# 1314wu/kvazaar

Hardware: AMD Instinct MI355X
Metric: Mblocks/s (SAD8/SATD8/DCT32) per GPU (higher is better)
Workload: dtype u8

## Files before the change

kvazaar_amd/csrc/api.hip:

```cpp
#include "kvz_hip_internal.h"

#include <atomic>
#include <cstdio>
#include <cstdlib>
#include <cstring>
#include <string>
#include <mutex>

namespace kvzhip {

constexpr int KVZ_MAX_DEVICES = 64;
struct dev_ctx {
  std::atomic<bool> ready{false};
  int num_cus = 256;
  hipStream_t stream = nullptr;
  char name[256] = "";
};
static std::mutex g_mu;
static dev_ctx g_ctx[KVZ_MAX_DEVICES];
static std::atomic<int> g_default_dev{-1};
static thread_local int t_dev = -1;
static thread_local char g_err[512] = "";

struct tune_entry { const char *key; std::atomic<int> value; };
static tune_entry g_tune[] = { { "sad_wgs_per_cu", {-1} }, { "satd8_wgs_per_cu", {-1} }, { "dct32_wgs_per_cu", {-1} },
                               { "idct32_wgs_per_cu", {-1} }, { "dct_wgs_per_cu", {-1} }, { "qr32_wgs_per_cu", {-1} },
                               { "qr_wgs_per_cu", {-1} }, { "dct16_wgs_per_cu", {-1} }, { "idct16_wgs_per_cu", {-1} },
                               { "qr16_wgs_per_cu", {-1} }, { "qr4_lane_kernel", {-1} },
                               { "sao_edge_fast", {-1} }, 
                               { "intra_rough_waves", {-1} }, { "pair_wave_kernel", {-1} }, { "qr4_wgs_per_cu", {-1} }, { "quant_wgs_per_cu", {-1} },
                               { "qr8_reg_kernel", {-1} }, { "qr8_wgs_per_cu", {-1} }, { "qr_tile_kernel", {-1} }, { "dct4_tile", {-1} }, { "dct4_wgs_per_cu", {-1} }, { "idct4_wgs_per_cu", {-1} },
                               { "wg_chunk_min_wgs", {-1} }, { "pair_satd_threads", {-1} }, { "qr8_tile_kernel", {-1} }, { "qr_tile_pipe", {-1} }, { "pipe", {-1} }, { "dct_pipe", {-1} }, { "sample8_wave", {-1} }, { "full_qsad", {-1} }, { "service_streams", {-1} }, { "service_inflight", {-1} }, { "service_workers", {-1} }, { "service_linger_us", {-1} }, { "service_life_ms", {-1} }, { "service_spin_us", {-1} }, { "service_ticket_base_k", {-1} }, { "service_push", {-1} }, { "service_nap_us", {-1} }, { "service_spin_crowded_us", {-1} } };
int tuning(const char *key, int dflt)
{
  for (auto &e : g_tune) if (!std::strcmp(e.key, key)) { const int v = e.value.load(std::memory_order_relaxed); return v >= 0 ? v : dflt; }
  return dflt;
}

int ctx_device() { return t_dev >= 0 ? t_dev : g_default_dev.load(std::memory_order_acquire); }
bool ctx_ready()
{
  const int d = ctx_device();
  return d >= 0 && g_ctx[d].ready.load(std::memory_order_acquire);
}

bool ctx_enter()
{
  const int d = ctx_device();
  if (d < 0 || !g_ctx[d].ready.load(std::memory_order_acquire)) return false;
  int cur = -1;
  if (hipGetDevice(&cur) != hipSuccess || cur != d) {
    if (hipSetDevice(d) != hipSuccess) return false;
  }
  return true;
}
// ... 390 lines not shown
```

kvazaar_amd/csrc/frac_core.h:

```cpp
#pragma once
#include "kvz_hip_internal.h"
#include "satd_regs.h"

namespace kvzhip {

static __constant__ __attribute__((aligned(8))) signed char c_luma_filter[4][8] = {
  { 0, 0, 0, 64, 0, 0, 0, 0 }, { -1, 4, -10, 58, 17, -5, 1, 0 }, { -1, 4, -11, 40, 40, -11, 4, -1 }, { 0, 1, -5, 17, 58, -10, 4, -1 } };

struct refplane_t { const u8 *p; u32 stride; int w, h; };

__device__ __forceinline__ u8 ref_px(const refplane_t &r, int x, int y)
{
  return r.p[(size_t)clampi(y, 0, r.h - 1) * r.stride + clampi(x, 0, r.w - 1)];
}

__device__ __forceinline__ u8 round_clip16(i16 sample) { return fast_clip16((i16)(((int)sample + 32) >> 6)); }

#define FR_HS 65

static __constant__ signed char c_sq_x[9] = { 0, -1, 1, 0, 0, -1, 1, -1, 1 };
static __constant__ signed char c_sq_y[9] = { 0, 0, 0, -1, 1, -1, -1, 1, 1 };

template <int MAXW>
struct frac_geom {
// ... 7 lines not shown
  static constexpr int H_OFF = (P_BYTES + CUR_BYTES + 15) & ~15;
  static constexpr int TOTAL = H_OFF + 4 * H_ELEMS * 2 + 32;
};

struct frac_vcoef { u32 c[4][2][2][5]; };
__host__ __device__ constexpr u32 frac_pack16(int lo, int hi) { return ((u32)lo & 0xffffu) | ((u32)hi << 16); }
__host__ __device__ constexpr frac_vcoef frac_make_vcoef()
{
  constexpr int f[4][8] = { { 0, 0, 0, 256, 0, 0, 0, 0 }, { -4, 16, -40, 232, 68, -20, 4, 0 }, { -4, 16, -44, 160, 160, -44, 16, -4 },
                            { 0, 4, -20, 68, 232, -40, 16, -4 } };
  frac_vcoef t = {};
  for (int fy = 0; fy < 4; ++fy)
    for (int i = 0; i < 5; ++i) {
      const u32 aligned = i < 4 ? frac_pack16(f[fy][2 * i], f[fy][2 * i + 1]) : 0u;
      const u32 shifted = frac_pack16(i > 0 ? f[fy][2 * i - 1] : 0, i < 4 ? f[fy][2 * i] : 0);
      const u32 late = i > 0 ? frac_pack16(f[fy][2 * i - 2], f[fy][2 * i - 1]) : 0u;
      t.c[fy][0][0][i] = aligned; t.c[fy][0][1][i] = shifted;
      t.c[fy][1][0][i] = shifted; t.c[fy][1][1][i] = late;
    }
  return t;
}
static __constant__ const frac_vcoef c_frac_vcoef = frac_make_vcoef();

__device__ __forceinline__ v2s frac_round_clip_pair(int acc_even, int acc_odd)
{
  const v2s sft = as_v2s(__builtin_amdgcn_perm((u32)acc_odd, (u32)acc_even, 0x06050201u));
  const v2s r32 = { 32, 32 }, six = { 6, 6 }, zero = { 0, 0 }, top = { 255, 255 };
  v2s t = __builtin_elementwise_add_sat(sft, r32) >> six;
  t = __builtin_elementwise_max(t, zero);
  return __builtin_elementwise_min(t, top);
}

struct frac_no_cost {
  __device__ __forceinline__ u32 cost(int, int, int, u32 &bits) const { bits = 0; return 0; }
  __device__ __forceinline__ bool within(int, int) const { return true; }
};
struct frac_result { int mvx, mvy; u32 cost, bitcost; u32 cost0; };

template <int MAXW, int T, bool WAVE, class MVC, int FW = 0, int FH = 0>
__device__ __forceinline__ frac_result search_frac_core(int tid, u8 *lds, const u8 *__restrict__ pic, u32 pic_stride, const refplane_t &ref,
                                                        const kvz_hip_block_pair &d, int fme_level, const MVC &mvc,
                                                        u32 *__restrict__ out, i32 *__restrict__ best)
{
  typedef frac_geom<MAXW> G;
  u8 *s_p = lds, *s_cur = s_p + G::P_BYTES;
  u32 *s_h = (u32 *)(lds + G::H_OFF);
  u32 *s_cost = s_h + 4 * (G::H_ELEMS / 2);
  int *s_sel = (int *)(s_cost + 4);
  auto sync = [&]() { if (WAVE) wave_lds_fence(); else __syncthreads(); };

  const int w = FW ? FW : d.width, h = FH ? FH : d.height;
  const int pw = w + 8, ph = h + 8;
  if (d.x2 - 4 >= 0 && d.x2 + w + 4 <= ref.w && d.y2 - 4 >= 0 && d.y2 + h + 4 <= ref.h) {
    const int pw4 = pw >> 2;
    const u8 *src = ref.p + (size_t)(d.y2 - 4) * ref.stride + (d.x2 - 4);
    for (int i = tid; i < pw4 * ph; i += T) {
      const int y = i / pw4, x = (i - y * pw4) * 4;
      u32 v;
      __builtin_memcpy(&v, src + (size_t)y * ref.stride + x, 4);
      *(u32 *)(s_p + y * G::PS + x) = v;
    }
  } else {
    for (int i = tid; i < pw * ph; i += T) {
      const int y = i / pw, x = i - y * pw;
      s_p[y * G::PS + x] = ref_px(ref, d.x2 - 4 + x, d.y2 - 4 + y);
// ... 112 lines not shown
#pragma unroll
      for (int j = 0; j < 8; ++j) {
        const u32 *cj = col + j * (G::HT >> 1);
        a0[j] = 0; a1[j] = 0;
#pragma unroll
        for (int t = 0; t < 5; ++t) {
          const v2s pr = as_v2s(cj[t]);
          a0[j] = __builtin_amdgcn_sdot2(pr, as_v2s(c0[t]), a0[j], false);
          a1[j] = __builtin_amdgcn_sdot2(pr, as_v2s(c1[t]), a1[j], false);
        }
      }
      v2s dd[2][4];
#pragma unroll
      for (int jj = 0; jj < 4; ++jj) {
        const u32 cw0 = cur[jj >> 1], cw1 = cur[2 + (jj >> 1)];
        dd[0][jj] = ((jj & 1) ? unpack_hi(cw0) : unpack_lo(cw0)) - frac_round_clip_pair(a0[2 * jj], a0[2 * jj + 1]);
        dd[1][jj] = ((jj & 1) ? unpack_hi(cw1) : unpack_lo(cw1)) - frac_round_clip_pair(a1[2 * jj], a1[2 * jj + 1]);
      }
      add_cost(k, satd8_quad_part_diff(dd, m1, m2));
    }
    sync();
  };

  auto score_step8 = [&](int pat, int ox, int oy, int scale) {
    const int g = tid & 3, pp = (tid >> 2) & 3, k = tid >> 4;
    const int sx = (int)((0x8858u >> (2 * (pat + k - 1))) & 3u) - 1, sy = (int)((0xa085u >> (2 * (pat + k - 1))) & 3u) - 1;
    const int qx = ox + scale * sx, qy = oy + scale * sy;
    const int fx = qx & 3, fy = qy & 3, cx = qx >> 2, ry = qy >> 2;
    const int slot = fx == 0 ? 0 : fx == 2 ? 1 : (sx > 0 ? 3 : 2);
    const int y0 = 2 * pp, b = y0 + ry + 1, par = b & 1;
    u32 c0[5], c1[5];
#pragma unroll
    for (int t = 0; t < 5; ++t) { c0[t] = c_frac_vcoef.c[fy][par][0][t]; c1[t] = c_frac_vcoef.c[fy][par][1][t]; }
    const u32 *col = s_h + slot * (G::H_ELEMS / 2) + ((2 * g + cx + 1) * G::HT >> 1) + (b >> 1);
    int a0[2], a1[2];
#pragma unroll
    for (int j = 0; j < 2; ++j) {
      const u32 *cj = col + j * (G::HT >> 1);
      a0[j] = 0; a1[j] = 0;
#pragma unroll
      for (int t = 0; t < 5; ++t) {
        const v2s pr = as_v2s(cj[t]);
        a0[j] = __builtin_amdgcn_sdot2(pr, as_v2s(c0[t]), a0[j], false);
        a1[j] = __builtin_amdgcn_sdot2(pr, as_v2s(c1[t]), a1[j], false);
      }
    }
    const u8 *a = s_cur + y0 * G::CS + 2 * g;
    const u32 cw0 = *(const unsigned short *)a, cw1 = *(const unsigned short *)(a + G::CS);
    const v2s r0 = unpack_lo(cw0) - frac_round_clip_pair(a0[0], a0[1]), r1 = unpack_lo(cw1) - frac_round_clip_pair(a1[0], a1[1]);
    const short s4 = (tid & 4) ? (short)-1 : (short)1, s8 = (tid & 8) ? (short)-1 : (short)1;
    const v2s m4 = { s4, s4 }, m8 = { s8, s8 };
    v2s v[2] = { r0 + r1, r0 - r1 };
    u32 acc = 0;
#pragma unroll
    for (int i = 0; i < 2; ++i) {
      v2s t = dpp_v2s<0xB1>(v[i]);
      v2s u = v[i] * m1 + t;
      t = dpp_v2s<0x4E>(u);
      u = u * m2 + t;
      t = dpp_xor4_v2s(u);
      u = u * m4 + t;
      t = dpp_v2s<0x128>(u);
      u = u * m8 + t;
      acc = abs_last_stage(u, acc);
    }
    acc = group_sum<16>(acc);
    if ((tid & 15) == 0) s_cost[k] = (acc + 2) >> 2;
    sync();
  };
  constexpr bool SPLIT8 = WAVE && T == 64 && FW == 8 && FH == 8;
  constexpr bool SPLIT16 = WAVE && T == 64 && FW == 16 && FH == 16;
  auto score_any = [&](int pat, int ox, int oy, int scale) {
    if constexpr (SPLIT8) score_step8(pat, ox, oy, scale); else score_step(pat, ox, oy, scale);
  };

  if constexpr (SPLIT8 || SPLIT16) {
    const int g = tid & 3, pp = (tid >> 2) & 3, sb = SPLIT16 ? tid >> 4 : 0, y0 = (sb >> 1) * 8 + 2 * pp, x0 = (sb & 1) * 8 + 2 * g;
    const u8 *a = s_cur + y0 * G::CS + x0, *bq = s_p + (4 + y0) * G::PS + 4 + x0;
    const u32 cw0 = *(const unsigned short *)a, cw1 = *(const unsigned short *)(a + G::CS);
    const u32 pw0 = *(const unsigned short *)bq, pw1 = *(const unsigned short *)(bq + G::PS);
    const v2s r0 = unpack_lo(cw0) - unpack_lo(pw0), r1 = unpack_lo(cw1) - unpack_lo(pw1);
    const short s4 = (tid & 4) ? (short)-1 : (short)1, s8 = (tid & 8) ? (short)-1 : (short)1;
    const v2s m4 = { s4, s4 }, m8 = { s8, s8 };
    v2s v[2] = { r0 + r1, r0 - r1 };
    u32 acc = 0;
#pragma unroll
    for (int i = 0; i < 2; ++i) {
      v2s t = dpp_v2s<0xB1>(v[i]);
      v2s u = v[i] * m1 + t;
      t = dpp_v2s<0x4E>(u);
      u = u * m2 + t;
      t = dpp_xor4_v2s(u);
      u = u * m4 + t;
      t = dpp_v2s<0x128>(u);
      u = u * m8 + t;
      acc = abs_last_stage(u, acc);
    }
    acc = (group_sum<16>(acc) + 2) >> 2;
    if (SPLIT16) acc = group_sum<64>((tid & 15) == 0 ? acc : 0u);
    if (tid == 0) s_cost[0] = acc;
    sync();
  } else {
    score_integer();
  }
  int mx = d.x2 - d.x1, my = d.y2 - d.y1;
  u32 best_bitcost = 0;
  u32 best_cost = s_cost[0];
  if (out && tid == 0) out[0] = best_cost;
  best_cost += mvc.cost(mx, my, 2, best_bitcost);
  const u32 cost0 = best_cost;
  mx *= 2; my *= 2;

  if (fme_level > 0) hor_planes(0, 0, 2, 1);
  sync();

  int best_index = 0, pat = 1;
  for (int step = 0; step < fme_level; ++step) {
    if (step < 2) {
      score_any(pat, 0, 0, 2);
    } else {
      const int hx = s_sel[0], hy = s_sel[1];
      if (step == 2) {
        hor_planes((2 * hx - 1) & 3, 2, (2 * hx + 1) & 3, 3);
        sync();
      }
      score_any(pat, 2 * hx, 2 * hy, 1);
    }
    const int mv_shift = step < 2 ? 1 : 0;
    const int lj = tid & 3;
    const int lpx = mx + (int)((0x8858u >> (2 * (pat + lj - 1))) & 3u) - 1, lpy = my + (int)((0xa085u >> (2 * (pat + lj - 1))) & 3u) - 1;
    u32 lbits = 0;
    const u32 lraw = s_cost[lj];
    const int lok = mvc.within(lpx * (1 << mv_shift), lpy * (1 << mv_shift)) ? 1 : 0;
    const u32 lcost = lraw + mvc.cost(lpx, lpy, mv_shift, lbits);
    if (out && tid < 4) out[(step >= 2 ? 8 : 0) + pat + tid] = lraw;
#pragma unroll
    for (int j = 0; j < 4; ++j) {
      const u32 cj = (u32)__builtin_amdgcn_readlane((int)lcost, j), bj = (u32)__builtin_amdgcn_readlane((int)lbits, j);
      if (!__builtin_amdgcn_readlane(lok, j)) continue;
      if (cj < best_cost) { best_cost = cj; best_bitcost = bj; best_index = pat + j; }
    }
    pat += 4;
    if (step == 1 || step == fme_level - 1) {
      if (best && tid == 0 && step == 3) best[1] = best_index;
      mx += c_sq_x[best_index]; my += c_sq_y[best_index];
      if (step == (fme_level - 1 < 1 ? fme_level - 1 : 1)) {
        if (best && tid == 0) best[0] = best_index;
        mx *= 2; my *= 2;
        sync();
        if (tid == 0) { s_sel[0] = c_sq_x[best_index]; s_sel[1] = c_sq_y[best_index]; }
        best_index = 0; pat = 1;
      }
    }
    sync();
  }
  frac_result res = { mx, my, best_cost, best_bitcost, cost0 };
  return res;
}

__device__ __forceinline__ bool frac_shape_ok(int w, int h)
// ... 6 lines not shown
```

kvazaar_amd/csrc/ipol.hip:

```cpp
#include "kvz_hip_internal.h"
#include "frac_core.h"

using namespace kvzhip;

__constant__ signed char c_chroma_filter[8][4] = {
  { 0, 64, 0, 0 }, { -2, 58, 10, -2 }, { -4, 54, 16, -2 }, { -6, 46, 28, -4 },
  { -4, 36, 36, -4 }, { -4, 28, 46, -6 }, { -2, 16, 54, -4 }, { -2, 10, 58, -2 } };


template <int TAPS, int MAXW> struct sample_geom {
  static constexpr int WS = MAXW + TAPS;
  static constexpr int WIN_BYTES = (MAXW + TAPS) * WS;
  static constexpr int HP = (MAXW + TAPS) / 2 + 1;
  static constexpr int HOR_DWORDS = MAXW * HP > (MAXW + TAPS - 1) * MAXW / 2 ? MAXW * HP : (MAXW + TAPS - 1) * MAXW / 2 + 1;
};
template <int TAPS, bool OUT14, int MAXW, int T, bool WAVE>
__device__ __forceinline__ void sample_core_fast(int tid, u8 *s_win, u32 *s_hor, const kvz_hip_ipol_block &b, size_t o, void *__restrict__ dst)
{
  typedef sample_geom<TAPS, MAXW> G;
  constexpr int HALF = TAPS / 2;
  const int w = b.width, h = b.height, wh = h + TAPS - 1;
  const signed char *hf = TAPS == 8 ? c_luma_filter[b.mv_frac_x & 3] : c_chroma_filter[b.mv_frac_x & 7];
  const signed char *vf = TAPS == 8 ? c_luma_filter[b.mv_frac_y & 3] : c_chroma_filter[b.mv_frac_y & 7];
  u32 h0 = 0, h1 = 0;
// ... 244 lines not shown
}

template <int TAPS, bool OUT14>
__global__ __launch_bounds__(256) void sample_small_kernel(refplane_t ref, const kvz_hip_ipol_block *__restrict__ blocks, size_t count,
                                                           const unsigned long long *__restrict__ out_offsets, void *__restrict__ dst, int kvz_sample8_wave)
{
  __shared__ __attribute__((aligned(16))) u8 s_win[4][sample_geom<TAPS, 16>::WIN_BYTES];
  __shared__ __attribute__((aligned(16))) i16 s_hor[4][2 * sample_geom<TAPS, 16>::HOR_DWORDS];
  const int wv = __builtin_amdgcn_readfirstlane(threadIdx.x >> 6);
  const size_t i = (size_t)blockIdx.x * 4 + wv;
  if (i >= count) return;
  const kvz_hip_ipol_block b = blocks[i];
  if (b.width < 1 || b.height < 1 || b.width > 16 || b.height > 16) return;
  if (TAPS == 8 && b.width == 8 && b.height == 8 && kvz_sample8_wave) {
    sample8x8_luma_wave<OUT14>(threadIdx.x & 63, s_win[wv], (u32 *)s_hor[wv], ref, b, (size_t)out_offsets[i], dst);
    return;
  }
  sample_core<TAPS, OUT14, 16, 64, true>(threadIdx.x & 63, s_win[wv], s_hor[wv], ref, b, (size_t)out_offsets[i], dst);
}


__global__ __launch_bounds__(256) void search_frac_big_kernel(const u8 *__restrict__ pic, u32 pic_stride, refplane_t ref,
                                                              const kvz_hip_block_pair *__restrict__ pairs, size_t count, unsigned chunk,
                                                              u32 *__restrict__ costs, i32 *__restrict__ best)
{
  __shared__ __attribute__((aligned(16))) u8 lds[frac_geom<64>::TOTAL];
  __shared__ unsigned long long s_mask;
  const int tid = threadIdx.x;
  const size_t first = (size_t)blockIdx.x * chunk;
  auto mine = [&](size_t i) {
    const int w = pairs[i].width, h = pairs[i].height;
    return !frac_shape_ok(w, h) || w > 32 || h > 32;
  };
  unsigned long long mask = chunk == 1 ? (unsigned long long)mine(first) : wg_chunk_mask(&s_mask, first, chunk, count, mine);
  while (mask) {
    const size_t i = first + (unsigned)__builtin_ctzll(mask);
    mask &= mask - 1;
    const kvz_hip_block_pair d = pairs[i];
    if (!frac_shape_ok(d.width, d.height)) {
      if (tid < 17) costs[i * 17 + tid] = 0xffffffffu;
      if (tid < 2) best[i * 2 + tid] = -1;
      continue;
    }
    search_frac_core<64, 256, false>(tid, lds, pic, pic_stride, ref, d, 4, frac_no_cost(), costs + i * 17, best + i * 2);
    __syncthreads();
  }
}

__global__ __launch_bounds__(256) void search_frac_small_kernel(const u8 *__restrict__ pic, u32 pic_stride, refplane_t ref,
                                                                const kvz_hip_block_pair *__restrict__ pairs, size_t count,
                                                                u32 *__restrict__ costs, i32 *__restrict__ best)
{
  __shared__ __attribute__((aligned(16))) u8 lds[4][(frac_geom<16>::TOTAL + 15) & ~15];
  const int wv = __builtin_amdgcn_readfirstlane(threadIdx.x >> 6);
  const size_t i = (size_t)blockIdx.x * 4 + wv;
  if (i >= count) return;
  const kvz_hip_block_pair d = pairs[i];
  if (!frac_shape_ok(d.width, d.height) || d.width > 16 || d.height > 16) return;
  const int lane = threadIdx.x & 63;
  if (d.width == 8 && d.height == 8)
    search_frac_core<16, 64, true, frac_no_cost, 8, 8>(lane, lds[wv], pic, pic_stride, ref, d, 4, frac_no_cost(), costs + i * 17, best + i * 2);
  else if (d.width == 16 && d.height == 16)
    search_frac_core<16, 64, true, frac_no_cost, 16, 16>(lane, lds[wv], pic, pic_stride, ref, d, 4, frac_no_cost(), costs + i * 17, best + i * 2);
  else
    search_frac_core<16, 64, true, frac_no_cost>(lane, lds[wv], pic, pic_stride, ref, d, 4, frac_no_cost(), costs + i * 17, best + i * 2);
}

__global__ __launch_bounds__(128) void search_frac_medium_kernel(const u8 *__restrict__ pic, u32 pic_stride, refplane_t ref,
                                                                 const kvz_hip_block_pair *__restrict__ pairs, size_t count,
                                                                 u32 *__restrict__ costs, i32 *__restrict__ best)
{
  __shared__ __attribute__((aligned(16))) u8 lds[2][(frac_geom<32>::TOTAL + 15) & ~15];
  const int wv = __builtin_amdgcn_readfirstlane(threadIdx.x >> 6);
  const size_t i = (size_t)blockIdx.x * 2 + wv;
  if (i >= count) return;
  const kvz_hip_block_pair d = pairs[i];
  if (!frac_shape_ok(d.width, d.height) || d.width > 32 || d.height > 32 || (d.width <= 16 && d.height <= 16)) return;
  const int lane = threadIdx.x & 63;
  if (d.width == 32 && d.height == 32)
    search_frac_core<32, 64, true, frac_no_cost, 32, 32>(lane, lds[wv], pic, pic_stride, ref, d, 4, frac_no_cost(), costs + i * 17, best + i * 2);
  else
    search_frac_core<32, 64, true, frac_no_cost>(lane, lds[wv], pic, pic_stride, ref, d, 4, frac_no_cost(), costs + i * 17, best + i * 2);
}

__global__ __launch_bounds__(256) void bipred_cost_kernel(const u8 *__restrict__ pic, u32 pic_stride, int pic_w, int pic_h,
                                                         refplane_t ref0, refplane_t ref1, const kvz_hip_bipred_cand *__restrict__ cands,
                                                         u32 *__restrict__ costs)
{
  __shared__ __attribute__((aligned(16))) u8 s_win[sample_geom<8, 64>::WIN_BYTES];
  __shared__ __attribute__((aligned(16))) i16 s_hor[2 * sample_geom<8, 64>::HOR_DWORDS];
  __shared__ __attribute__((aligned(16))) i16 s_s[2][64 * 64];
  __shared__ __attribute__((aligned(16))) u8 s_pred[64 * 64], s_cur[64 * 64];
  __shared__ u32 s_cost;
  const kvz_hip_bipred_cand &c = cands[blockIdx.x];
  const int tid = threadIdx.x, w = c.width, h = c.height;
  if (!frac_shape_ok(w, h) || c.x < 0 || c.y < 0 || c.x + w > pic_w || c.y + h > pic_h) {
    if (tid == 0) costs[blockIdx.x] = 0xffffffffu;
    return;
  }
  if (tid == 0) s_cost = 0;
  for (int k = 0; k < 2; ++k) {
    const refplane_t &ref = k ? ref1 : ref0;
    const int mvx = k ? c.mv1[0] : c.mv0[0], mvy = k ? c.mv1[1] : c.mv0[1];
    const int ix = c.x + (mvx >> 2), iy = c.y + (mvy >> 2);
    if ((mvx & 3) || (mvy & 3)) {
// ... 189 lines not shown
int kvz_hip_sample_luma_batch(const kvz_hip_pixel *ref, uint32_t ref_stride, int ref_w, int ref_h,
                              const kvz_hip_ipol_block *blocks, const uint64_t *out_offsets, size_t count,
                              int out_14bit, void *dst, kvz_hip_stream s)
{
  return sample_launch(true, ref, ref_stride, ref_w, ref_h, blocks, out_offsets, count, out_14bit, dst, s);
}

int kvz_hip_sample_chroma_batch(const kvz_hip_pixel *ref, uint32_t ref_stride, int ref_w, int ref_h,
                                const kvz_hip_ipol_block *blocks, const uint64_t *out_offsets, size_t count,
                                int out_14bit, void *dst, kvz_hip_stream s)
{
  return sample_launch(false, ref, ref_stride, ref_w, ref_h, blocks, out_offsets, count, out_14bit, dst, s);
}

int kvz_hip_search_frac_batch(const kvz_hip_pixel *pic, uint32_t pic_stride, const kvz_hip_pixel *ref, uint32_t ref_stride,
                              int ref_w, int ref_h, const kvz_hip_block_pair *pairs, size_t count,
                              uint32_t *costs, int32_t *best, kvz_hip_stream s)
{
  KVZ_CHECK_CTX();
  if (!pic || !ref || !pairs || !costs || !best || ref_w <= 0 || ref_h <= 0) return kvzhip::invalid_arg(__func__);
  if (count == 0) return KVZ_HIP_OK;
  if (count > 0x7fffffffu) return kvzhip::invalid_arg(__func__);
  refplane_t r = { ref, ref_stride, ref_w, ref_h };
  hipLaunchKernelGGL(search_frac_small_kernel, dim3((unsigned)((count + 3) / 4)), dim3(256), 0, ctx_stream(s), pic, pic_stride, r, pairs, count, costs, best);
  KVZ_CHECK_LAUNCH("search_frac_small_kernel");
  const unsigned chunk = wg_chunk(count);
  hipLaunchKernelGGL(search_frac_big_kernel, dim3((unsigned)((count + chunk - 1) / chunk)), dim3(256), 0, ctx_stream(s), pic, pic_stride, r, pairs, count, chunk, costs, best);
  KVZ_CHECK_LAUNCH("search_frac_big_kernel");
  hipLaunchKernelGGL(search_frac_medium_kernel, dim3((unsigned)((count + 1) / 2)), dim3(128), 0, ctx_stream(s), pic, pic_stride, r, pairs, count, costs, best);
  KVZ_CHECK_LAUNCH("search_frac_medium_kernel");
  return KVZ_HIP_OK;
}

int kvz_hip_bipred_cost_batch(const kvz_hip_pixel *pic, uint32_t pic_stride, int pic_w, int pic_h,
                              const kvz_hip_pixel *ref0, uint32_t ref0_stride, const kvz_hip_pixel *ref1, uint32_t ref1_stride,
                              int ref_w, int ref_h, const kvz_hip_bipred_cand *cands, size_t count, uint32_t *costs, kvz_hip_stream s)
{
  KVZ_CHECK_CTX();
  if (!pic || !ref0 || !ref1 || !cands || !costs || pic_w <= 0 || pic_h <= 0 || ref_w <= 0 || ref_h <= 0) return kvzhip::invalid_arg(__func__);
  if (count == 0) return KVZ_HIP_OK;
  if (count > 0x7fffffffu) return kvzhip::invalid_arg(__func__);
  const refplane_t r0 = { ref0, ref0_stride, ref_w, ref_h }, r1 = { ref1, ref1_stride, ref_w, ref_h };
  hipLaunchKernelGGL(bipred_cost_kernel, dim3((unsigned)count), dim3(256), 0, ctx_stream(s), pic, pic_stride, pic_w, pic_h, r0, r1, cands, costs);
  KVZ_CHECK_LAUNCH("bipred_cost_kernel");
  return KVZ_HIP_OK;
}

}
```

kvazaar_amd/csrc/kvz_hip_internal.h:

```cpp
#pragma once

#include <hip/hip_runtime.h>
#include <stddef.h>
#include <stdint.h>

#include "../../include/kvz_hip.h"

typedef uint8_t u8;
typedef uint32_t u32;
typedef int16_t i16;
typedef int32_t i32;

namespace kvzhip {

int ctx_device();
bool ctx_ready();
bool ctx_enter();
hipStream_t ctx_stream(kvz_hip_stream s);
void set_error(const char *what, hipError_t e);
void set_error_msg(const char *what);
int invalid_arg(const char *entry);
int num_cus();
int tuning(const char *key, int dflt);
int stream_on_current_device(kvz_hip_stream s, const char *entry);

int copy_rects_launch(const kvz_hip_rect_copy *rects, int n, hipStream_t st, const char *entry);

#define KVZ_CHECK_CTX()                         \
  do {                                          \
    if (!kvzhip::ctx_enter()) {                 \
      if (kvz_hip_init(-1) != KVZ_HIP_OK || !kvzhip::ctx_enter()) return KVZ_HIP_ERR_NO_DEVICE; \
    }                                           \
  } while (0)

#define KVZ_CHECK_LAUNCH(name)                               \
  do {                                                       \
    hipError_t e__ = hipGetLastError();                      \
    if (e__ != hipSuccess) {                                 \
      kvzhip::set_error(name, e__);                          \
      return KVZ_HIP_ERR_RUNTIME;                            \
    }                                                        \
  } while (0)

static inline size_t wg_cap(long long per_cu) { return (size_t)num_cus() * (size_t)(per_cu > 0 ? per_cu : 1); }

static inline unsigned stream_grid(size_t work_items, unsigned items_per_block, unsigned max_blocks_per_cu = 128)
// ... 69 lines not shown
```

kvazaar_amd/csrc/me_search.hip:

```cpp
#include "me_search_core.h"

using namespace kvzhip;

namespace {

template <bool MULTI>
__device__ __forceinline__ bool pick_planes(const u8 *__restrict__ &pic, refplane_t &ref, const kvz_hip_me_pu &pu, int n_planes)
{
  if (!MULTI) return true;
  const int k = pu.pad >> 2;
  if (k < 0 || k >= n_planes) return false;
  pic = reinterpret_cast<const u8 *const *>(pic)[k];
  ref.p = reinterpret_cast<const u8 *const *>(ref.p)[k];
  return true;
}

template <int T, bool CONSTR, bool MULTI = false>
__global__ __launch_bounds__(T) void search_pu_big_kernel(const u8 *__restrict__ pic, u32 pic_stride, int pic_w, int pic_h, refplane_t ref,
                                                            const kvz_hip_me_pu *__restrict__ pus, kvz_hip_me_params prm,
                                                            kvz_hip_me_result *__restrict__ out)
{
  __shared__ __attribute__((aligned(16))) u8 lds[frac_geom<64>::TOTAL];
  __shared__ me_shared sh;
  const kvz_hip_me_pu &pu = pus[blockIdx.x];
// ... 96 lines not shown
  if (prm_v.tile_w == 0 && prm_v.tile_h == 0) { prm_v.tile_x = 0; prm_v.tile_y = 0; prm_v.tile_w = pic_w; prm_v.tile_h = pic_h; }
  if (prm_v.mv_constraint < 0 || prm_v.mv_constraint > 4 || prm_v.tile_x < 0 || prm_v.tile_y < 0 || prm_v.tile_w <= 0 || prm_v.tile_h <= 0 ||
      prm_v.tile_x + prm_v.tile_w > pic_w || prm_v.tile_y + prm_v.tile_h > pic_h || (prm_v.wpp_owf && ((prm_v.tile_x & 63) || (prm_v.tile_y & 63)))) {
    set_error_msg("kvz_hip_search_pu_batch: mv_constraint must be 0..4 and the tile must lie inside the picture (origin a multiple of 64 when wpp_owf is set: its rule counts LCUs from there)");
    return KVZ_HIP_ERR_INVALID;
  }
  params = &prm_v;
  if (count == 0) return KVZ_HIP_OK;
  if (count > 0x7fffffffu) return kvzhip::invalid_arg(__func__);
  hipStream_t st = ctx_stream(s);
  const refplane_t r = { ref, ref_stride, ref_w, ref_h };
  if (params->mv_rdo) {
    if (n_planes) { set_error_msg("kvz_hip_search_pu_multi_batch: mv_rdo is a one-picture path"); return KVZ_HIP_ERR_INVALID; }
    if (!params->cabac || params->n_cabac < 1 || params->refs_before < 1 || params->refs_before > 16 || params->ref_idx < 0 || params->ref_idx >= 16) {
      set_error_msg("kvz_hip_search_pu_batch: mv_rdo needs the cabac snapshots (device array of n_cabac >= 1), refs_before 1..16 and ref_idx 0..15");
      return KVZ_HIP_ERR_INVALID;
    }
    hipLaunchKernelGGL(search_pu_rdo_kernel, dim3((unsigned)count), dim3(256), 0, st, pic, pic_stride, pic_w, pic_h, r, pus, *params, results);
    KVZ_CHECK_LAUNCH("search_pu_rdo_kernel");
    return KVZ_HIP_OK;
  }
  const int classes = (params->size_classes & 7) ? (params->size_classes & 7) : 7;
  prm_v.size_classes = classes;
  prm_v.n_cabac = n_planes;
  const bool constrained = params->wpp_owf != 0 || params->mv_constraint != 0;
  if (n_planes) {
    if (constrained) launch_classes<true, true>(classes, pic, pic_stride, pic_w, pic_h, r, pus, count, *params, results, st);
    else launch_classes<false, true>(classes, pic, pic_stride, pic_w, pic_h, r, pus, count, *params, results, st);
  } else {
    if (constrained) launch_classes<true, false>(classes, pic, pic_stride, pic_w, pic_h, r, pus, count, *params, results, st);
    else launch_classes<false, false>(classes, pic, pic_stride, pic_w, pic_h, r, pus, count, *params, results, st);
  }
  KVZ_CHECK_LAUNCH("search_pu kernels");
  return KVZ_HIP_OK;
}

extern "C" int kvz_hip_search_pu_batch(const kvz_hip_pixel *pic, uint32_t pic_stride, int pic_w, int pic_h,
                                       const kvz_hip_pixel *ref, uint32_t ref_stride, int ref_w, int ref_h,
                                       const kvz_hip_me_pu *pus, size_t count, const kvz_hip_me_params *params,
                                       kvz_hip_me_result *results, kvz_hip_stream s)
{
  return search_pu_launch(pic, pic_stride, pic_w, pic_h, ref, ref_stride, ref_w, ref_h, 0, pus, count, params, results, s);
}

extern "C" int kvz_hip_search_pu_multi_batch(const kvz_hip_pixel *const *pics, uint32_t pic_stride, int pic_w, int pic_h,
                                             const kvz_hip_pixel *const *refs, uint32_t ref_stride, int ref_w, int ref_h, int n_planes,
// ... 8 lines not shown
```

kvazaar_amd/csrc/me_search_core.h:

```cpp
#pragma once
#include "frac_core.h"
#include "me_cost.h"
#include "serve_ring.h"
#include <type_traits>

namespace kvzhip {

static __constant__ signed char c_large_hex[9][2] = { { 0, 0 }, { 1, -2 }, { 2, 0 }, { 1, 2 }, { -1, 2 }, { -2, 0 }, { -1, -2 }, { 1, -2 }, { 2, 0 } };
static __constant__ signed char c_small_hex[9][2] = { { 0, 0 }, { 0, -1 }, { -1, 0 }, { 1, 0 }, { 0, 1 }, { -1, -1 }, { 1, -1 }, { -1, 1 }, { 1, 1 } };
static __constant__ signed char c_diamond[5][2] = { { 0, -1 }, { 1, 0 }, { 0, 1 }, { -1, 0 }, { 0, 0 } };
static __constant__ signed char c_et_hex[7][2] = { { 0, -1 }, { -1, 0 }, { 0, 1 }, { 1, 0 }, { 0, -1 }, { -1, 0 }, { 0, 0 } };

constexpr int ME_GROUP = 64;
struct me_shared { u32 sad[ME_GROUP]; int cx[ME_GROUP], cy[ME_GROUP]; };

constexpr int FULL_OUT = 32;
constexpr int FULL_MAX_WINDOWS = 7;

template <bool CONSTR, bool QSAD, int T>
__device__ __forceinline__ void full_search_wg(int tid, u8 *lds, int lds_bytes, me_shared *sh, const u8 *__restrict__ pic, u32 pic_stride,
                                               const refplane_t &ref, const kvz_hip_me_pu &pu, const kvz_hip_me_params &prm)
{
  const me_cost_model_t<false, CONSTR> mvc(pu, prm);
  const int w = pu.width, h = pu.height, R = prm.search_range, side = 2 * R + 1;
// ... 489 lines not shown
      const int start = best_index == 1 ? 6 : (best_index == 8 ? 1 : best_index - 1);
      mvx += c_large_hex[best_index][0]; mvy += c_large_hex[best_index][1];
      best_index = 0;
      sync();
      for (int i = 0; i < 3; ++i) set_cand(i, mvx + c_large_hex[start + i][0], mvy + c_large_hex[start + i][1]);
      group_sads(3);
      const int hit = decide(3);
      if (hit >= 0) best_index = start + hit;
    }
    sync();
    for (int i = 1; i < 9; ++i) set_cand(i - 1, mvx + c_small_hex[i][0], mvy + c_small_hex[i][1]);
    group_sads(8);
    decide(8);
  }

  int mv_x = best_x * 4, mv_y = best_y * 4;
  const u32 int_cost = best_cost, int_bits = best_bits;
  u32 cost0 = 0xffffffffu;
  if (best_cost != 0xffffffffu) {
    sync();
    const kvz_hip_block_pair d = { pu.x, pu.y, pu.x + best_x, pu.y + best_y, w, h };
    const u32 beat = (!BOTH && prm.cost_to_beat) ? prm.cost_to_beat[pu_index] : 0xffffffffu;
    const int level = __builtin_amdgcn_readfirstlane(best_cost < beat ? prm.fme_level : 0);
    const frac_result fr = search_frac_core<MAXW, T, WAVE, me_cost_model_t<RDO, CONSTR>, FW, FH>(tid, lds, pic, pic_stride, ref, d, level, mvc, (u32 *)nullptr, (i32 *)nullptr);
    best_cost = fr.cost;
    cost0 = fr.cost0;
    if (level > 0) { mv_x = fr.mvx; mv_y = fr.mvy; best_bits = fr.bitcost; }
  }

  if (BOTH) {
    if (tid == 0) {
      serve_result *so = reinterpret_cast<serve_result *>(out);
      kvz_hip_me_result r;
      u32 unused;
      r.mv[0] = mv_x; r.mv[1] = mv_y;
      r.cost = best_cost; r.bitcost = best_bits;
      int m = mvc.merge_match(mv_x, mv_y);
      r.merged = m >= 0;
      r.merge_idx = m >= 0 ? m : mvc.n_merge;
      r.mv_cand = m >= 0 ? 0 : mvc.select_cand(mv_x, mv_y, unused);
      r.reserved = 0;
      so->frac = r;
      r.mv[0] = best_x * 4; r.mv[1] = best_y * 4;
      r.cost = cost0; r.bitcost = int_bits;
      m = mvc.merge_match(best_x * 4, best_y * 4);
      r.merged = m >= 0;
      r.merge_idx = m >= 0 ? m : mvc.n_merge;
// ... 43 lines not shown
```

Before: 24300.

## Score all eight half-pel ring candidates in one shared pass

```diff
diff --git a/kvazaar_amd/csrc/api.hip b/kvazaar_amd/csrc/api.hip
--- a/kvazaar_amd/csrc/api.hip
+++ b/kvazaar_amd/csrc/api.hip
@@ -30,7 +30,7 @@
                                { "sao_edge_fast", {-1} }, 
                                { "intra_rough_waves", {-1} }, { "pair_wave_kernel", {-1} }, { "qr4_wgs_per_cu", {-1} }, { "quant_wgs_per_cu", {-1} },
                                { "qr8_reg_kernel", {-1} }, { "qr8_wgs_per_cu", {-1} }, { "qr_tile_kernel", {-1} }, { "dct4_tile", {-1} }, { "dct4_wgs_per_cu", {-1} }, { "idct4_wgs_per_cu", {-1} },
-                               { "wg_chunk_min_wgs", {-1} }, { "pair_satd_threads", {-1} }, { "qr8_tile_kernel", {-1} }, { "qr_tile_pipe", {-1} }, { "pipe", {-1} }, { "dct_pipe", {-1} }, { "sample8_wave", {-1} }, { "full_qsad", {-1} }, { "service_streams", {-1} }, { "service_inflight", {-1} }, { "service_workers", {-1} }, { "service_linger_us", {-1} }, { "service_life_ms", {-1} }, { "service_spin_us", {-1} }, { "service_ticket_base_k", {-1} }, { "service_push", {-1} }, { "service_nap_us", {-1} }, { "service_spin_crowded_us", {-1} } };
+                               { "wg_chunk_min_wgs", {-1} }, { "pair_satd_threads", {-1} }, { "qr8_tile_kernel", {-1} }, { "qr_tile_pipe", {-1} }, { "pipe", {-1} }, { "dct_pipe", {-1} }, { "sample8_wave", {-1} }, { "full_qsad", {-1} }, { "frac_shared_half", {-1} }, { "service_streams", {-1} }, { "service_inflight", {-1} }, { "service_workers", {-1} }, { "service_linger_us", {-1} }, { "service_life_ms", {-1} }, { "service_spin_us", {-1} }, { "service_ticket_base_k", {-1} }, { "service_push", {-1} }, { "service_nap_us", {-1} }, { "service_spin_crowded_us", {-1} } };
 int tuning(const char *key, int dflt)
 {
   for (auto &e : g_tune) if (!std::strcmp(e.key, key)) { const int v = e.value.load(std::memory_order_relaxed); return v >= 0 ? v : dflt; }
diff --git a/kvazaar_amd/csrc/frac_core.h b/kvazaar_amd/csrc/frac_core.h
--- a/kvazaar_amd/csrc/frac_core.h
+++ b/kvazaar_amd/csrc/frac_core.h
@@ -53,13 +53,27 @@
 }
 static __constant__ const frac_vcoef c_frac_vcoef = frac_make_vcoef();
 
-__device__ __forceinline__ v2s frac_round_clip_pair(int acc_even, int acc_odd)
-{
-  const v2s sft = as_v2s(__builtin_amdgcn_perm((u32)acc_odd, (u32)acc_even, 0x06050201u));
+__device__ __forceinline__ v2s frac_round_clip_pk(v2s sft)
+{
   const v2s r32 = { 32, 32 }, six = { 6, 6 }, zero = { 0, 0 }, top = { 255, 255 };
   v2s t = __builtin_elementwise_add_sat(sft, r32) >> six;
   t = __builtin_elementwise_max(t, zero);
   return __builtin_elementwise_min(t, top);
+}
+__device__ __forceinline__ v2s frac_round_clip_pair(int acc_even, int acc_odd)
+{
+  return frac_round_clip_pk(as_v2s(__builtin_amdgcn_perm((u32)acc_odd, (u32)acc_even, 0x06050201u)));
+}
+
+__device__ __forceinline__ void frac_half_rows3(const u32 *cj, int &r0, int &r1, int &r2)
+{
+  constexpr u32 A0 = frac_pack16(-4, 16), A1 = frac_pack16(-44, 160), A2 = frac_pack16(160, -44), A3 = frac_pack16(16, -4);
+  constexpr u32 S0 = frac_pack16(0, -4), S1 = frac_pack16(16, -44), S2 = frac_pack16(160, 160), S3 = frac_pack16(-44, 16), S4 = frac_pack16(-4, 0);
+  const v2s p0 = as_v2s(cj[0]), p1 = as_v2s(cj[1]), p2 = as_v2s(cj[2]), p3 = as_v2s(cj[3]), p4 = as_v2s(cj[4]);
+  auto dot = [](v2s a, u32 c, int acc) { return __builtin_amdgcn_sdot2(a, as_v2s(c), acc, false); };
+  r0 = dot(p3, A3, dot(p2, A2, dot(p1, A1, dot(p0, A0, 0))));
+  r1 = dot(p4, S4, dot(p3, S3, dot(p2, S2, dot(p1, S1, dot(p0, S0, 0)))));
+  r2 = dot(p4, A3, dot(p3, A2, dot(p2, A1, dot(p1, A0, 0))));
 }
 
 struct frac_no_cost {
@@ -68,10 +82,10 @@
 };
 struct frac_result { int mvx, mvy; u32 cost, bitcost; u32 cost0; };
 
-template <int MAXW, int T, bool WAVE, class MVC, int FW = 0, int FH = 0>
+template <int MAXW, int T, bool WAVE, class MVC, int FW = 0, int FH = 0, bool RING = WAVE>
 __device__ __forceinline__ frac_result search_frac_core(int tid, u8 *lds, const u8 *__restrict__ pic, u32 pic_stride, const refplane_t &ref,
                                                         const kvz_hip_block_pair &d, int fme_level, const MVC &mvc,
-                                                        u32 *__restrict__ out, i32 *__restrict__ best)
+                                                        u32 *__restrict__ out, i32 *__restrict__ best, bool two_passes = false)
 {
   typedef frac_geom<MAXW> G;
   u8 *s_p = lds, *s_cur = s_p + G::P_BYTES;
@@ -230,32 +244,7 @@
     sync();
   };
 
-  auto score_step8 = [&](int pat, int ox, int oy, int scale) {
-    const int g = tid & 3, pp = (tid >> 2) & 3, k = tid >> 4;
-    const int sx = (int)((0x8858u >> (2 * (pat + k - 1))) & 3u) - 1, sy = (int)((0xa085u >> (2 * (pat + k - 1))) & 3u) - 1;
-    const int qx = ox + scale * sx, qy = oy + scale * sy;
-    const int fx = qx & 3, fy = qy & 3, cx = qx >> 2, ry = qy >> 2;
-    const int slot = fx == 0 ? 0 : fx == 2 ? 1 : (sx > 0 ? 3 : 2);
-    const int y0 = 2 * pp, b = y0 + ry + 1, par = b & 1;
-    u32 c0[5], c1[5];
-#pragma unroll
-    for (int t = 0; t < 5; ++t) { c0[t] = c_frac_vcoef.c[fy][par][0][t]; c1[t] = c_frac_vcoef.c[fy][par][1][t]; }
-    const u32 *col = s_h + slot * (G::H_ELEMS / 2) + ((2 * g + cx + 1) * G::HT >> 1) + (b >> 1);
-    int a0[2], a1[2];
-#pragma unroll
-    for (int j = 0; j < 2; ++j) {
-      const u32 *cj = col + j * (G::HT >> 1);
-      a0[j] = 0; a1[j] = 0;
-#pragma unroll
-      for (int t = 0; t < 5; ++t) {
-        const v2s pr = as_v2s(cj[t]);
-        a0[j] = __builtin_amdgcn_sdot2(pr, as_v2s(c0[t]), a0[j], false);
-        a1[j] = __builtin_amdgcn_sdot2(pr, as_v2s(c1[t]), a1[j], false);
-      }
-    }
-    const u8 *a = s_cur + y0 * G::CS + 2 * g;
-    const u32 cw0 = *(const unsigned short *)a, cw1 = *(const unsigned short *)(a + G::CS);
-    const v2s r0 = unpack_lo(cw0) - frac_round_clip_pair(a0[0], a0[1]), r1 = unpack_lo(cw1) - frac_round_clip_pair(a1[0], a1[1]);
+  auto satd_split16 = [&](v2s r0, v2s r1) {
     const short s4 = (tid & 4) ? (short)-1 : (short)1, s8 = (tid & 8) ? (short)-1 : (short)1;
     const v2s m4 = { s4, s4 }, m8 = { s8, s8 };
     v2s v[2] = { r0 + r1, r0 - r1 };
@@ -272,14 +261,121 @@
       u = u * m8 + t;
       acc = abs_last_stage(u, acc);
     }
-    acc = group_sum<16>(acc);
-    if ((tid & 15) == 0) s_cost[k] = (acc + 2) >> 2;
+    return (group_sum<16>(acc) + 2) >> 2;
+  };
+
+  auto score_step8 = [&](int pat, int ox, int oy, int scale) {
+    const int g = tid & 3, pp = (tid >> 2) & 3, k = tid >> 4;
+    const int sx = (int)((0x8858u >> (2 * (pat + k - 1))) & 3u) - 1, sy = (int)((0xa085u >> (2 * (pat + k - 1))) & 3u) - 1;
+    const int qx = ox + scale * sx, qy = oy + scale * sy;
+    const int fx = qx & 3, fy = qy & 3, cx = qx >> 2, ry = qy >> 2;
+    const int slot = fx == 0 ? 0 : fx == 2 ? 1 : (sx > 0 ? 3 : 2);
+    const int y0 = 2 * pp, b = y0 + ry + 1, par = b & 1;
+    u32 c0[5], c1[5];
+#pragma unroll
+    for (int t = 0; t < 5; ++t) { c0[t] = c_frac_vcoef.c[fy][par][0][t]; c1[t] = c_frac_vcoef.c[fy][par][1][t]; }
+    const u32 *col = s_h + slot * (G::H_ELEMS / 2) + ((2 * g + cx + 1) * G::HT >> 1) + (b >> 1);
+    int a0[2], a1[2];
+#pragma unroll
+    for (int j = 0; j < 2; ++j) {
+      const u32 *cj = col + j * (G::HT >> 1);
+      a0[j] = 0; a1[j] = 0;
+#pragma unroll
+      for (int t = 0; t < 5; ++t) {
+        const v2s pr = as_v2s(cj[t]);
+        a0[j] = __builtin_amdgcn_sdot2(pr, as_v2s(c0[t]), a0[j], false);
+        a1[j] = __builtin_amdgcn_sdot2(pr, as_v2s(c1[t]), a1[j], false);
+      }
+    }
+    const u8 *a = s_cur + y0 * G::CS + 2 * g;
+    const u32 cw0 = *(const unsigned short *)a, cw1 = *(const unsigned short *)(a + G::CS);
+    const v2s r0 = unpack_lo(cw0) - frac_round_clip_pair(a0[0], a0[1]), r1 = unpack_lo(cw1) - frac_round_clip_pair(a1[0], a1[1]);
+    const u32 acc = satd_split16(r0, r1);
+    if ((tid & 15) == 0) s_cost[k] = acc;
     sync();
   };
   constexpr bool SPLIT8 = WAVE && T == 64 && FW == 8 && FH == 8;
   constexpr bool SPLIT16 = WAVE && T == 64 && FW == 16 && FH == 16;
   auto score_any = [&](int pat, int ox, int oy, int scale) {
     if constexpr (SPLIT8) score_step8(pat, ox, oy, scale); else score_step(pat, ox, oy, scale);
+  };
+
+  auto score_ring = [&]() {
+    if (tid < 8) s_cost[tid] = 0;
+    sync();
+    for (int i = tid; i < 4 * n8 * 4; i += T) {
+      const int q = i >> 2, grp = q / n8, sb = q - grp * n8, by = sb / w8, bx = sb - by * w8;
+      const int y0 = by * 8 + 2 * p;
+      const u8 *a = s_cur + y0 * G::CS + bx * 8;
+      u32 cur[4];
+      __builtin_memcpy(&cur[0], a, 4); __builtin_memcpy(&cur[1], a + 4, 4); __builtin_memcpy(&cur[2], a + G::CS, 4); __builtin_memcpy(&cur[3], a + G::CS + 4, 4);
+      v2s da[2][4], db[2][4];
+      if (grp < 3) {
+        const u32 *col = s_h + (grp == 2 ? 0 : G::H_ELEMS / 2) + ((bx * 8 + (grp == 0 ? 0 : 1)) * G::HT >> 1) + (y0 >> 1);
+#pragma unroll
+        for (int jj = 0; jj < 4; ++jj) {
+          int r0[2], r1[2], r2[2];
+#pragma unroll
+          for (int j = 0; j < 2; ++j) frac_half_rows3(col + (2 * jj + j) * (G::HT >> 1), r0[j], r1[j], r2[j]);
+          da[0][jj] = frac_round_clip_pair(r0[0], r0[1]);
+          da[1][jj] = db[0][jj] = frac_round_clip_pair(r1[0], r1[1]);
+          db[1][jj] = frac_round_clip_pair(r2[0], r2[1]);
+        }
+      } else {
+        const u32 *col = s_h + G::H_ELEMS / 2 + (bx * 8 * G::HT >> 1) + (y0 >> 1) + 2;
+        u32 v[9];
+#pragma unroll
+        for (int j = 0; j < 9; ++j) v[j] = col[j * (G::HT >> 1)];
+#pragma unroll
+        for (int jj = 0; jj < 4; ++jj) {
+          da[0][jj] = frac_round_clip_pk(as_v2s(__builtin_amdgcn_perm(v[2 * jj + 1], v[2 * jj], 0x05040100u)));
+          da[1][jj] = frac_round_clip_pk(as_v2s(__builtin_amdgcn_perm(v[2 * jj + 1], v[2 * jj], 0x07060302u)));
+          db[0][jj] = frac_round_clip_pk(as_v2s(__builtin_amdgcn_perm(v[2 * jj + 2], v[2 * jj + 1], 0x05040100u)));
+          db[1][jj] = frac_round_clip_pk(as_v2s(__builtin_amdgcn_perm(v[2 * jj + 2], v[2 * jj + 1], 0x07060302u)));
+        }
+      }
+#pragma unroll
+      for (int jj = 0; jj < 4; ++jj) {
+        const u32 cw0 = cur[jj >> 1], cw1 = cur[2 + (jj >> 1)];
+        const v2s c0 = (jj & 1) ? unpack_hi(cw0) : unpack_lo(cw0), c1 = (jj & 1) ? unpack_hi(cw1) : unpack_lo(cw1);
+        da[0][jj] = c0 - da[0][jj]; da[1][jj] = c1 - da[1][jj];
+        db[0][jj] = c0 - db[0][jj]; db[1][jj] = c1 - db[1][jj];
+      }
+      const int ka = grp == 0 ? 4 : grp == 1 ? 5 : grp == 2 ? 2 : 0;
+      add_cost(ka, satd8_quad_part_diff(da, m1, m2));
+      add_cost(grp == 3 ? 1 : ka + (grp == 2 ? 1 : 2), satd8_quad_part_diff(db, m1, m2));
+    }
+    sync();
+  };
+
+  auto score_ring8 = [&]() {
+    const int g = tid & 3, pp = (tid >> 2) & 3, grp = tid >> 4, y0 = 2 * pp;
+    const u8 *a = s_cur + y0 * G::CS + 2 * g;
+    const v2s c0 = unpack_lo(*(const unsigned short *)a), c1 = unpack_lo(*(const unsigned short *)(a + G::CS));
+    v2s a0, a1, b0, b1;
+    if (grp < 3) {
+      const u32 *col = s_h + (grp == 2 ? 0 : G::H_ELEMS / 2) + ((2 * g + (grp == 0 ? 0 : 1)) * G::HT >> 1) + (y0 >> 1);
+      int r0[2], r1[2], r2[2];
+#pragma unroll
+      for (int j = 0; j < 2; ++j) frac_half_rows3(col + j * (G::HT >> 1), r0[j], r1[j], r2[j]);
+      a0 = frac_round_clip_pair(r0[0], r0[1]);
+      a1 = b0 = frac_round_clip_pair(r1[0], r1[1]);
+      b1 = frac_round_clip_pair(r2[0], r2[1]);
+    } else {
+      const u32 *col = s_h + G::H_ELEMS / 2 + (2 * g * G::HT >> 1) + (y0 >> 1) + 2;
+      const u32 v0 = col[0], v1 = col[G::HT >> 1], v2 = col[2 * (G::HT >> 1)];
+      a0 = frac_round_clip_pk(as_v2s(__builtin_amdgcn_perm(v1, v0, 0x05040100u)));
+      a1 = frac_round_clip_pk(as_v2s(__builtin_amdgcn_perm(v1, v0, 0x07060302u)));
+      b0 = frac_round_clip_pk(as_v2s(__builtin_amdgcn_perm(v2, v1, 0x05040100u)));
+      b1 = frac_round_clip_pk(as_v2s(__builtin_amdgcn_perm(v2, v1, 0x07060302u)));
+    }
+    const u32 sa = satd_split16(c0 - a0, c1 - a1), sb = satd_split16(c0 - b0, c1 - b1);
+    if ((tid & 15) == 0) {
+      const int ka = grp == 0 ? 4 : grp == 1 ? 5 : grp == 2 ? 2 : 0;
+      s_cost[ka] = sa;
+      s_cost[grp == 3 ? 1 : ka + (grp == 2 ? 1 : 2)] = sb;
+    }
+    sync();
   };
 
   if constexpr (SPLIT8 || SPLIT16) {
@@ -288,23 +384,7 @@
     const u32 cw0 = *(const unsigned short *)a, cw1 = *(const unsigned short *)(a + G::CS);
     const u32 pw0 = *(const unsigned short *)bq, pw1 = *(const unsigned short *)(bq + G::PS);
     const v2s r0 = unpack_lo(cw0) - unpack_lo(pw0), r1 = unpack_lo(cw1) - unpack_lo(pw1);
-    const short s4 = (tid & 4) ? (short)-1 : (short)1, s8 = (tid & 8) ? (short)-1 : (short)1;
-    const v2s m4 = { s4, s4 }, m8 = { s8, s8 };
-    v2s v[2] = { r0 + r1, r0 - r1 };
-    u32 acc = 0;
-#pragma unroll
-    for (int i = 0; i < 2; ++i) {
-      v2s t = dpp_v2s<0xB1>(v[i]);
-      v2s u = v[i] * m1 + t;
-      t = dpp_v2s<0x4E>(u);
-      u = u * m2 + t;
-      t = dpp_xor4_v2s(u);
-      u = u * m4 + t;
-      t = dpp_v2s<0x128>(u);
-      u = u * m8 + t;
-      acc = abs_last_stage(u, acc);
-    }
-    acc = (group_sum<16>(acc) + 2) >> 2;
+    u32 acc = satd_split16(r0, r1);
     if (SPLIT16) acc = group_sum<64>((tid & 15) == 0 ? acc : 0u);
     if (tid == 0) s_cost[0] = acc;
     sync();
@@ -319,12 +399,16 @@
   const u32 cost0 = best_cost;
   mx *= 2; my *= 2;
 
+  const bool ring = RING && fme_level >= 2 && !two_passes;
   if (fme_level > 0) hor_planes(0, 0, 2, 1);
   sync();
 
   int best_index = 0, pat = 1;
-  for (int step = 0; step < fme_level; ++step) {
-    if (step < 2) {
+  for (int step = ring ? 1 : 0; step < fme_level; ++step) {
+    const int ncand = (ring && step == 1) ? 8 : 4;
+    if (ncand == 8) {
+      if constexpr (!RING) {} else if constexpr (SPLIT8) score_ring8(); else score_ring();
+    } else if (step < 2) {
       score_any(pat, 0, 0, 2);
     } else {
       const int hx = s_sel[0], hy = s_sel[1];
@@ -335,15 +419,17 @@
       score_any(pat, 2 * hx, 2 * hy, 1);
     }
     const int mv_shift = step < 2 ? 1 : 0;
-    const int lj = tid & 3;
+    constexpr int NC = RING ? 8 : 4;
+    const int lj = tid & (NC - 1);
     const int lpx = mx + (int)((0x8858u >> (2 * (pat + lj - 1))) & 3u) - 1, lpy = my + (int)((0xa085u >> (2 * (pat + lj - 1))) & 3u) - 1;
     u32 lbits = 0;
     const u32 lraw = s_cost[lj];
     const int lok = mvc.within(lpx * (1 << mv_shift), lpy * (1 << mv_shift)) ? 1 : 0;
     const u32 lcost = lraw + mvc.cost(lpx, lpy, mv_shift, lbits);
-    if (out && tid < 4) out[(step >= 2 ? 8 : 0) + pat + tid] = lraw;
-#pragma unroll
-    for (int j = 0; j < 4; ++j) {
+    if (out && tid < (RING ? ncand : 4)) out[(step >= 2 ? 8 : 0) + pat + tid] = lraw;
+#pragma unroll
+    for (int j = 0; j < NC; ++j) {
+      if (NC > 4 && j >= ncand) break;
       const u32 cj = (u32)__builtin_amdgcn_readlane((int)lcost, j), bj = (u32)__builtin_amdgcn_readlane((int)lbits, j);
       if (!__builtin_amdgcn_readlane(lok, j)) continue;
       if (cj < best_cost) { best_cost = cj; best_bitcost = bj; best_index = pat + j; }
diff --git a/kvazaar_amd/csrc/ipol.hip b/kvazaar_amd/csrc/ipol.hip
--- a/kvazaar_amd/csrc/ipol.hip
+++ b/kvazaar_amd/csrc/ipol.hip
@@ -290,7 +290,7 @@
 
 __global__ __launch_bounds__(256) void search_frac_big_kernel(const u8 *__restrict__ pic, u32 pic_stride, refplane_t ref,
                                                               const kvz_hip_block_pair *__restrict__ pairs, size_t count, unsigned chunk,
-                                                              u32 *__restrict__ costs, i32 *__restrict__ best)
+                                                              u32 *__restrict__ costs, i32 *__restrict__ best, int two_passes)
 {
   __shared__ __attribute__((aligned(16))) u8 lds[frac_geom<64>::TOTAL];
   __shared__ unsigned long long s_mask;
@@ -310,14 +310,14 @@
       if (tid < 2) best[i * 2 + tid] = -1;
       continue;
     }
-    search_frac_core<64, 256, false>(tid, lds, pic, pic_stride, ref, d, 4, frac_no_cost(), costs + i * 17, best + i * 2);
+    search_frac_core<64, 256, false>(tid, lds, pic, pic_stride, ref, d, 4, frac_no_cost(), costs + i * 17, best + i * 2, two_passes != 0);
     __syncthreads();
   }
 }
 
 __global__ __launch_bounds__(256) void search_frac_small_kernel(const u8 *__restrict__ pic, u32 pic_stride, refplane_t ref,
                                                                 const kvz_hip_block_pair *__restrict__ pairs, size_t count,
-                                                                u32 *__restrict__ costs, i32 *__restrict__ best)
+                                                                u32 *__restrict__ costs, i32 *__restrict__ best, int two_passes)
 {
   __shared__ __attribute__((aligned(16))) u8 lds[4][(frac_geom<16>::TOTAL + 15) & ~15];
   const int wv = __builtin_amdgcn_readfirstlane(threadIdx.x >> 6);
@@ -327,16 +327,16 @@
   if (!frac_shape_ok(d.width, d.height) || d.width > 16 || d.height > 16) return;
   const int lane = threadIdx.x & 63;
   if (d.width == 8 && d.height == 8)
-    search_frac_core<16, 64, true, frac_no_cost, 8, 8>(lane, lds[wv], pic, pic_stride, ref, d, 4, frac_no_cost(), costs + i * 17, best + i * 2);
+    search_frac_core<16, 64, true, frac_no_cost, 8, 8>(lane, lds[wv], pic, pic_stride, ref, d, 4, frac_no_cost(), costs + i * 17, best + i * 2, two_passes != 0);
   else if (d.width == 16 && d.height == 16)
-    search_frac_core<16, 64, true, frac_no_cost, 16, 16>(lane, lds[wv], pic, pic_stride, ref, d, 4, frac_no_cost(), costs + i * 17, best + i * 2);
+    search_frac_core<16, 64, true, frac_no_cost, 16, 16>(lane, lds[wv], pic, pic_stride, ref, d, 4, frac_no_cost(), costs + i * 17, best + i * 2, two_passes != 0);
   else
-    search_frac_core<16, 64, true, frac_no_cost>(lane, lds[wv], pic, pic_stride, ref, d, 4, frac_no_cost(), costs + i * 17, best + i * 2);
+    search_frac_core<16, 64, true, frac_no_cost>(lane, lds[wv], pic, pic_stride, ref, d, 4, frac_no_cost(), costs + i * 17, best + i * 2, two_passes != 0);
 }
 
 __global__ __launch_bounds__(128) void search_frac_medium_kernel(const u8 *__restrict__ pic, u32 pic_stride, refplane_t ref,
                                                                  const kvz_hip_block_pair *__restrict__ pairs, size_t count,
-                                                                 u32 *__restrict__ costs, i32 *__restrict__ best)
+                                                                 u32 *__restrict__ costs, i32 *__restrict__ best, int two_passes)
 {
   __shared__ __attribute__((aligned(16))) u8 lds[2][(frac_geom<32>::TOTAL + 15) & ~15];
   const int wv = __builtin_amdgcn_readfirstlane(threadIdx.x >> 6);
@@ -346,9 +346,9 @@
   if (!frac_shape_ok(d.width, d.height) || d.width > 32 || d.height > 32 || (d.width <= 16 && d.height <= 16)) return;
   const int lane = threadIdx.x & 63;
   if (d.width == 32 && d.height == 32)
-    search_frac_core<32, 64, true, frac_no_cost, 32, 32>(lane, lds[wv], pic, pic_stride, ref, d, 4, frac_no_cost(), costs + i * 17, best + i * 2);
+    search_frac_core<32, 64, true, frac_no_cost, 32, 32>(lane, lds[wv], pic, pic_stride, ref, d, 4, frac_no_cost(), costs + i * 17, best + i * 2, two_passes != 0);
   else
-    search_frac_core<32, 64, true, frac_no_cost>(lane, lds[wv], pic, pic_stride, ref, d, 4, frac_no_cost(), costs + i * 17, best + i * 2);
+    search_frac_core<32, 64, true, frac_no_cost>(lane, lds[wv], pic, pic_stride, ref, d, 4, frac_no_cost(), costs + i * 17, best + i * 2, two_passes != 0);
 }
 
 __global__ __launch_bounds__(256) void bipred_cost_kernel(const u8 *__restrict__ pic, u32 pic_stride, int pic_w, int pic_h,
@@ -584,12 +584,13 @@
   if (count == 0) return KVZ_HIP_OK;
   if (count > 0x7fffffffu) return kvzhip::invalid_arg(__func__);
   refplane_t r = { ref, ref_stride, ref_w, ref_h };
-  hipLaunchKernelGGL(search_frac_small_kernel, dim3((unsigned)((count + 3) / 4)), dim3(256), 0, ctx_stream(s), pic, pic_stride, r, pairs, count, costs, best);
+  const int two_passes = kvzhip::tuning("frac_shared_half", 1) ? 0 : 1;
+  hipLaunchKernelGGL(search_frac_small_kernel, dim3((unsigned)((count + 3) / 4)), dim3(256), 0, ctx_stream(s), pic, pic_stride, r, pairs, count, costs, best, two_passes);
   KVZ_CHECK_LAUNCH("search_frac_small_kernel");
   const unsigned chunk = wg_chunk(count);
-  hipLaunchKernelGGL(search_frac_big_kernel, dim3((unsigned)((count + chunk - 1) / chunk)), dim3(256), 0, ctx_stream(s), pic, pic_stride, r, pairs, count, chunk, costs, best);
+  hipLaunchKernelGGL(search_frac_big_kernel, dim3((unsigned)((count + chunk - 1) / chunk)), dim3(256), 0, ctx_stream(s), pic, pic_stride, r, pairs, count, chunk, costs, best, two_passes);
   KVZ_CHECK_LAUNCH("search_frac_big_kernel");
-  hipLaunchKernelGGL(search_frac_medium_kernel, dim3((unsigned)((count + 1) / 2)), dim3(128), 0, ctx_stream(s), pic, pic_stride, r, pairs, count, costs, best);
+  hipLaunchKernelGGL(search_frac_medium_kernel, dim3((unsigned)((count + 1) / 2)), dim3(128), 0, ctx_stream(s), pic, pic_stride, r, pairs, count, costs, best, two_passes);
   KVZ_CHECK_LAUNCH("search_frac_medium_kernel");
   return KVZ_HIP_OK;
 }
diff --git a/kvazaar_amd/csrc/kvz_hip_internal.h b/kvazaar_amd/csrc/kvz_hip_internal.h
--- a/kvazaar_amd/csrc/kvz_hip_internal.h
+++ b/kvazaar_amd/csrc/kvz_hip_internal.h
@@ -22,6 +22,7 @@
 int invalid_arg(const char *entry);
 int num_cus();
 int tuning(const char *key, int dflt);
+constexpr int FRAC_RING_TWO_PASSES = 8;
 int stream_on_current_device(kvz_hip_stream s, const char *entry);
 
 int copy_rects_launch(const kvz_hip_rect_copy *rects, int n, hipStream_t st, const char *entry);
diff --git a/kvazaar_amd/csrc/me_search.hip b/kvazaar_amd/csrc/me_search.hip
--- a/kvazaar_amd/csrc/me_search.hip
+++ b/kvazaar_amd/csrc/me_search.hip
@@ -142,6 +142,7 @@
   }
   const int classes = (params->size_classes & 7) ? (params->size_classes & 7) : 7;
   prm_v.size_classes = classes;
+  if (!kvzhip::tuning("frac_shared_half", 1)) prm_v.size_classes |= FRAC_RING_TWO_PASSES;
   prm_v.n_cabac = n_planes;
   const bool constrained = params->wpp_owf != 0 || params->mv_constraint != 0;
   if (n_planes) {
diff --git a/kvazaar_amd/csrc/me_search_core.h b/kvazaar_amd/csrc/me_search_core.h
--- a/kvazaar_amd/csrc/me_search_core.h
+++ b/kvazaar_amd/csrc/me_search_core.h
@@ -535,7 +535,8 @@
     const kvz_hip_block_pair d = { pu.x, pu.y, pu.x + best_x, pu.y + best_y, w, h };
     const u32 beat = (!BOTH && prm.cost_to_beat) ? prm.cost_to_beat[pu_index] : 0xffffffffu;
     const int level = __builtin_amdgcn_readfirstlane(best_cost < beat ? prm.fme_level : 0);
-    const frac_result fr = search_frac_core<MAXW, T, WAVE, me_cost_model_t<RDO, CONSTR>, FW, FH>(tid, lds, pic, pic_stride, ref, d, level, mvc, (u32 *)nullptr, (i32 *)nullptr);
+    const frac_result fr = search_frac_core<MAXW, T, WAVE, me_cost_model_t<RDO, CONSTR>, FW, FH, WAVE && !BOTH>(tid, lds, pic, pic_stride, ref, d, level, mvc, (u32 *)nullptr, (i32 *)nullptr,
+                                                                                                                 (prm.size_classes & FRAC_RING_TWO_PASSES) != 0);
     best_cost = fr.cost;
     cost0 = fr.cost0;
     if (level > 0) { mv_x = fr.mvx; mv_y = fr.mvy; best_bits = fr.bitcost; }
```

After: 24310 (median of 3 runs). Within noise of the previous version (+0.0%).
